# nikihowe/myriad

Hardware: AMD Instinct MI355X
Metric: converged trajopt solves/sec (batched), CARTPOLE collocation N=100 (higher is better)
Workload: dtype f64; 1 GPU; CARTPOLE HS collocation N=100, batch=4096 random x0 (weak), converged = status 0 and max|c|<=1e-8; global_batch=4096, parallelism=instances sharded over 1 GPU(s), one process per GPU

## Files before the change

myriad_amd/csrc/hs_solver_fused.h:

```cpp
#pragma once
#include <hip/hip_runtime.h>
#include "hs_solver_wave.h"

namespace myriad {

struct ParkArgs {
  int mode;
  int k1;
  const int* perm;
  const int* count;
  double* state;
  long stride;
  int fill;
  int shift;
  int* reached;
  int* cnt;
#ifdef MYR_SLOT_STAMPS
  long long* stamps;
#endif
};
constexpr int MYR_STATUS_PARKED_ = 5;
constexpr int SLOT_STAMP_WORDS = 64;

constexpr int PARK_BUCKETS = 256;
// ... 95 lines not shown
  __host__ __device__ static long off_mb(int N) { return off_hb(N) + (MLP ? (long)NodeMfma64::ntiles(npoints(N)) * NodeMfma64::HB_TILE : 0); }
  __host__ __device__ static long off_zlu(int N) { return off_mb(N) + (MLP ? (long)NodeMfma64::ntiles(npoints(N)) * NodeMfma64::MB_TILE : 0); }
  static constexpr bool FSEQ = (MYR_FWD_SEQ_NW > 0) && NW >= MYR_FWD_SEQ_NW && !MLP;
  static constexpr int FWS = NW * NW + NW;
  __host__ __device__ static long off_fw(int N) { return off_zlu(N) + (ZLU_GLOBAL ? 2L * npoints(N) * NW : 0); }
  __host__ __device__ static long scratch_doubles(int N) { return off_fw(N) + (FSEQ ? (long)N * FWS : 0); }
  static constexpr int NREC = NS + NS + NS * NS + NS * NU + NS;
  static constexpr int EXCH = NW * NW + NW * NC + NS * NC + NU * NC;
  static constexpr int NTOT = NW * NW + NW, NRED = 12;
  static constexpr int XCH = 2 * W * NREC + 2 * W * NTOT + 2 * W * 2 * NS + W * NRED + 8;
  static constexpr int NCH = W;
  static constexpr int NXB = TL ? NCH : (W > 1 ? 2 : 1);
  static constexpr int TL_TH1 = NCH * NC, TL_JN1 = (NCH - 1) * 4 * NW * NW;
  static constexpr int TL_TH = TL ? TL_TH1 + (NCH + 1) + 2 : 0, TL_JN = TL ? TL_JN1 : 0;
  __host__ __device__ static constexpr int lds_solver_doubles_z(int N, bool zlu_global) { return (zlu_global ? 2 : 4) * npoints(N) * NW + MLAM * N * NS + 6 * NW + XCH + NXB * EXCH + TL_TH + TL_JN + 8; }
  static constexpr bool ZLU_GLOBAL = (MLP && W == 2) ||
      (!MLP && (MYR_FWD_SEQ_NW > 0) && NW >= MYR_FWD_SEQ_NW && (long)lds_solver_doubles_z(100, false) * 8 > 40960L * W);
  __host__ __device__ static int lds_solver_doubles(int N) { return lds_solver_doubles_z(N, ZLU_GLOBAL); }
  __host__ __device__ static int lds_doubles(int N) { return lds_solver_doubles(N) + (MLP ? npoints(N) * NS + NodeTraits<Sys>::lds_doubles : 0); }
  __host__ __device__ static size_t lds_bytes(int N) { return (size_t)lds_doubles(N) * 8; }
  static constexpr int NSCAL = 48;
  static constexpr int PK_UNI = IpState<NS>::RECORD, PK_RES = PK_UNI + 1, PK_IT = PK_RES + 4;
  static_assert(PK_IT + 1 <= NSCAL, "record of a parked trajectory");
  __host__ __device__ static long park_doubles(int N) { return NSCAL + lds_solver_doubles(N) + (ZLU_GLOBAL ? 2L * npoints(N) * NW : 0); }

  struct Ctx {
    int N, K, n, lane, wave, tid;
    double h, h6, h8;
    double *z, *zL, *zU, *dz;
    double *hr, *st, *kg, *zr;
    double *fw;
    double *kgA, *kgB, *xA, *xB;
    double *sTh, *sJn;
    double *pt, *sF, *wl;
    double *hb, *mb;
    int nh, hidx;
    unsigned int gen;
    NodeBoard* board; int* coop_abort;
    double *pubx, *publam, *pubf;
    bool h_valid;
    const double *lb, *ub;
    bool uni;
    bool at_k1;
    SysParams<Sys> pp;
    bool term_pinned[NS];
    double *sLam, *sB, *sStash, *sTot, *sTr, *sRed, *sMisc, *sP, *sPc, *sTnu, *sKu;
#ifdef MYR_PHASE_TIMING
    long long tph[16], t0;
#endif
#ifdef MYR_TRACE
    int traj;
#endif
  };
  __device__ static inline long zi(const Ctx& c, int j, int comp) { return S::zi(c.K, j, comp); }
  __device__ static inline void use_set(Ctx& c, double* kg, double* x) {
    c.kg = kg; c.sP = x; c.sPc = x + NW * NW; c.sTnu = c.sPc + NW * NC; c.sKu = c.sTnu + NS * NC;
  }
  __device__ static inline void wsync() {
    __syncthreads();
  }
  template <int NV>
  __device__ static inline void wg_combine(Ctx& c, double* v, const int (&op)[NV]) {
    static_assert(NV <= NRED, "partial-sum slots");
    if constexpr (W > 1) {
#pragma unroll
      for (int i = 0; i < NV; ++i) c.sRed[c.wave * NRED + i] = v[i];
      __syncthreads();
#pragma unroll
      for (int i = 0; i < NV; ++i) {
        double r = c.sRed[i];
#pragma unroll
        for (int w = 1; w < W; ++w) {
          const double t = c.sRed[w * NRED + i];
          r = op[i] == 0 ? r + t : (op[i] == 1 ? (r > t ? r : t) : (r < t ? r : t));
        }
        v[i] = r;
      }
    } else { (void)c; (void)v; (void)op; }
  }

  __device__ static inline unsigned int& coop_seq(Ctx& c) { return reinterpret_cast<unsigned int*>(c.sMisc)[6]; }
  __device__ static inline unsigned int& coop_target(Ctx& c) { return reinterpret_cast<unsigned int*>(c.sMisc)[7]; }
  __device__ static inline bool coop_bounded(Ctx& c, unsigned int& spins) {
    if (++spins > MYR_COOP_SPIN_MAX || __hip_atomic_load(c.coop_abort, __ATOMIC_RELAXED, __HIP_MEMORY_SCOPE_AGENT) != 0) {
      if (spins > MYR_COOP_SPIN_MAX) __hip_atomic_store(c.coop_abort, 1, __ATOMIC_RELAXED, __HIP_MEMORY_SCOPE_AGENT);
      return true;
    }
    return false;
  }
  __device__ static inline void coop_refresh(Ctx& c) {
    if constexpr (MLP) {
      unsigned int* w = reinterpret_cast<unsigned int*>(c.sMisc) + 8;
      if (c.tid == 0) *w = __hip_atomic_load(&c.board->att, __ATOMIC_RELAXED, __HIP_MEMORY_SCOPE_AGENT) & 0xffffu;
      __syncthreads();
      const int a = __builtin_amdgcn_readfirstlane((int)*w);
      if (c.tid == 0) { COOP_TR(0, 100 + a); } if (c.tid == 64) { COOP_TR(11, 100 + a); } if (c.tid == 128) { COOP_TR(12, 100 + a); } if (c.tid == 192) { COOP_TR(13, 100 + a); }
      if (a != c.nh) { if (c.tid == 0) COOP_DBG(1, "[wg %d] owner: helpers %d -> %d\n", (int)blockIdx.x, c.nh, a); c.nh = a; c.h_valid = false; }
    } else (void)c;
  }
  template <int MODE>
  __device__ static inline void coop_post(Ctx& c, double alpha) {
    if constexpr (MLP) {
      if (MODE == 0) { for (int i = c.tid; i < c.n; i += NT) c.pubx[i] = fma(alpha, c.dz[i], c.z[i]); }
      if (MODE == 3 && !c.h_valid) { for (int i = c.tid; i < c.n; i += NT) c.pubx[i] = c.z[i]; }
      if (MODE == 4) { for (int i = c.tid; i < MLAM * c.N * NS; i += NT) c.publam[i] = c.sLam[i]; }
      if (c.tid == 0) COOP_TR(9, 1);
      coop_release();
// ... 132 lines not shown
            if (__hip_atomic_load(co.abort + 1, __ATOMIC_RELAXED, __HIP_MEMORY_SCOPE_AGENT) >= B) { quit = 1; COOP_DBG(32, "[wg %d] all finished: quit\n", (int)blockIdx.x); break; }
            __builtin_amdgcn_s_sleep(64);
            if (coop_bounded(c, spins)) { quit = 1; break; }
          }
          info[0] = found; info[1] = hid; info[2] = (int)seen; info[3] = quit | (int)(gen << 1);
          COOP_TR(5, found); COOP_TR(6, hid); COOP_TR(10, quit ? 999 : 0);
        }
        __syncthreads();
        const int found = __builtin_amdgcn_readfirstlane(info[0]), hid = __builtin_amdgcn_readfirstlane(info[1]);
        const unsigned int seen = (unsigned int)__builtin_amdgcn_readfirstlane(info[2]);
        const int quit_gen = __builtin_amdgcn_readfirstlane(info[3]);
        const int quit = quit_gen & 1;
        __syncthreads();
        if (quit) break;
        c.gen = (unsigned int)(quit_gen >> 1);
        double* so = scratch + (long)found * scratch_stride;
        c.pt = so + off_pt(c.N); c.hb = so + off_hb(c.N); c.mb = so + off_mb(c.N);
        c.board = co.boards + found; c.hidx = hid;
        c.pubx = co.pub + (long)found * co.pub_stride; c.publam = c.pubx + c.n; c.pubf = c.publam + MLAM * c.N * NS;
        coop_serve(c, seen);
      }
    } else (void)ha;
  }

  template <int MODE>
  __device__ static inline void node_pass(Ctx& c, double alpha) {
    if constexpr (MLP) {
#ifdef MYR_PHASE_TIMING
      const long long tn0_ = clock64();
#endif
      NodeMfma64::ArgsT<nd_lds> a;
      a.z = (const nd_lds*)c.z; a.dz = (const nd_lds*)c.dz; a.lam = (const nd_lds*)c.sLam; a.pt = (nd_glb*)c.pt;
      a.sF = (nd_lds*)c.sF;
      a.alpha = alpha; a.h6 = c.h6; a.h8 = c.h8; a.K = c.K; a.N = c.N;
      a.pf_f = PT_F; a.pf_a = PT_A; a.pf_b = PT_B; a.pf_d2 = PT_D2;
      a.t0 = c.wave; a.ts = W * (c.nh + 1);
      a.hb = (nd_glb*)c.hb; a.mb = (nd_glb*)c.mb; a.h_valid = c.h_valid ? 1 : 0;
      if (c.nh > 0) coop_post<MODE>(c, alpha);
      NodeMfma64::pass<MODE, nd_lds>((const nd_lds*)c.wl, a, c.lane);
      if (c.nh > 0) coop_wait<MODE>(c);
#ifdef MYR_PHASE_TIMING
      if (blockIdx.x == 0 && c.tid == 0) node_tph_[MODE] += clock64() - tn0_;
#endif
    } else { (void)c; (void)alpha; }
  }

  __device__ static inline void load_bounds(const Ctx& c, int j, double* l, double* u) {
    if (c.uni) {
      const nd_lds* b = (const nd_lds*)c.sB + ((j == 0) ? 0 : ((j == c.K - 1) ? 2 * NW : 4 * NW));
#pragma unroll
      for (int q = 0; q < NW; ++q) { l[q] = b[q]; u[q] = b[NW + q]; }
    } else {
#pragma unroll
      for (int q = 0; q < NW; ++q) { const long i = zi(c, j, q); l[q] = c.lb[i]; u[q] = c.ub[i]; }
    }
  }

  struct Step { bool on; double ap, ad, mu, ksig; };
  struct Acc { double f, cmax, cmin, sm, lg; int nm; };
  struct PRec { double x[NS], f[NS], A[NS * NS], B[NS * NU], own[NS]; };

  __device__ static inline void step_at(Ctx& c, const Step& st, int j, PRec&) {
    double bl[NW], bu[NW];
    load_bounds(c, j, bl, bu);
    const double iks = 1.0 / st.ksig;
#pragma unroll
    for (int q = 0; q < NW; ++q) {
      const long i = zi(c, j, q);
      const double l = bl[q], u = bu[q], zv = c.z[i], d = c.dz[i], zl = c.zL[i], zu = c.zU[i];
      const BoundKind k = bound_kind(l, u);
      const double zn = k.fr ? fma(st.ap, d, zv) : zv;
      const BoundMult m = bound_accept<true>(k, l, u, zv, zn, d, zl, zu, st.ad, st.mu, st.ksig, iks);
      c.z[i] = zn; c.zL[i] = m.zL; c.zU[i] = m.zU;
    }
  }

  __device__ static inline void lin_at(Ctx& c, const Step& st, int j, bool live, PRec& R, Acc& a) {
    typename S::VarBlk V;
    load_bounds(c, j, V.l, V.u);
    const double iks = 1.0 / st.ksig;
    double dv[NW];
#pragma unroll
    for (int q = 0; q < NW; ++q) {
      const long i = zi(c, j, q);
      V.z[q] = c.z[i]; V.zl[q] = c.zL[i]; V.zu[q] = c.zU[i];
      dv[q] = st.on ? c.dz[i] : 0.0;
    }
    if (st.on) {
#pragma unroll
      for (int q = 0; q < NW; ++q) {
        const long i = zi(c, j, q);
        const double l = V.l[q], u = V.u[q], zv = V.z[q], d = dv[q], zl = V.zl[q], zu = V.zu[q];
        const BoundKind k = bound_kind(l, u);
        const double zn = k.fr ? fma(st.ap, d, zv) : zv;
        const BoundMult m = bound_accept<true>(k, l, u, zv, zn, d, zl, zu, st.ad, st.mu, st.ksig, iks);
        V.z[q] = zn; V.zl[q] = m.zL; V.zu[q] = m.zU;
        if (live) { c.z[i] = V.z[q]; c.zL[i] = V.zl[q]; c.zU[i] = V.zu[q]; }
      }
    }
    double u_[NU], g, gw[NW];
#pragma unroll
    for (int q = 0; q < NS; ++q) R.x[q] = V.z[q];
#pragma unroll
    for (int q = 0; q < NU; ++q) u_[q] = V.z[NS + q];
    set_time<Sys>(c.pp.get(), tq(j, c.h));
    if constexpr (MLP) {
      const double* pt = c.pt + j;
      const int K = c.K;
#pragma unroll
      for (int q = 0; q < NS; ++q) R.f[q] = pt[(PT_F + q) * K];
#pragma unroll
      for (int q = 0; q < NS * NS; ++q) R.A[q] = pt[(PT_A + q) * K];
#pragma unroll
      for (int q = 0; q < NS * NU; ++q) R.B[q] = pt[(PT_B + q) * K];
      Sys::cost_grad(R.x, u_, c.pp.get(), &g, gw);
    } else
      Sys::lin(R.x, u_, c.pp.get(), R.f, R.A, R.B, &g, gw);
    const double wj = wq(c.K, j, c.h);
    if (TRAP && j == c.K - 1) fold_terminal<Sys>(R.x, u_, c.pp.get(), wj, g, gw);
    double cmax = a.cmax, cmin = a.cmin, sm = 0.0; int nm = 0;
    SlackLog sl;
#pragma unroll
    for (int q = 0; q < NW; ++q) {
      BoundTerms b = bound_terms(V.z[q], V.l[q], V.u[q], V.zl[q], V.zu[q], cmax, cmin);
      if (q < NS) R.own[q < NS ? q : 0] = wj * gw[q] + b.zlu;
      const BoundKind k = bound_kind(V.l[q], V.u[q]);
      mult_sum(k, V.zl[q], V.zu[q], sm, nm);
      sl.add(k, V.z[q], V.l[q], V.u[q]);
    }
    if (live) {
      a.cmax = cmax; a.cmin = cmin; a.sm += sm; a.nm += nm;
      a.lg -= sl.value();
      a.f += wj * g;
    }
  }

  struct BOut { double f, cmax, cmin, sm, lg, c1, cinf, lam_inf, sum_mult; int nm; };
  __device__ static void backward(Ctx& c, const Step& stp, const double* nuT, BOut& o) {
    using namespace detail;
    const int N = c.N, K = c.K, lane = c.lane;
    const double h6 = c.h6, h8 = c.h8;
    Acc acc{0.0, 0.0, INFINITY, 0.0, 0.0, 0};
    double c1 = 0, cinf = 0, li_ = 0, smu = 0;
    double piS[NS];
#pragma unroll
    for (int q = 0; q < NS; ++q) piS[q] = c.term_pinned[q] ? nuT[q] : 0.0;
    Step stp_ = stp;
    if constexpr (MLP) {
      if (stp.on) {
        Acc dummy{0.0, 0.0, INFINITY, 0.0, 0.0, 0};
        for (int j = c.tid; j < K; j += NT) { PRec R; step_at(c, stp, j, R); }
        (void)dummy;
        wsync();
        stp_.on = false;
      }
      node_pass<3>(c, 0.0);
      __builtin_amdgcn_fence(__ATOMIC_RELEASE, "workgroup");
      wsync();
    }
    int round = 0;
#ifdef MYR_PHASE_TIMING
    long long bw_t0_ = clock64();
#endif
    for (int r0 = N / 64; r0 >= 0; r0 -= W, ++round) {
      const int blk = r0 - c.wave;
      const int kr = blk >= 0 ? blk * 64 + 63 - lane : N + 1;
      const bool on_s = kr <= N, on = kr < N;
      const int k = on_s ? kr : N;
      PRec Rs, Rm, Re;
      lin_at(c, stp_, TRAP ? k : 2 * k, on_s, Rs, acc);
      if constexpr (!TRAP) lin_at(c, stp_, on ? 2 * k + 1 : 2 * k, on, Rm, acc);
      {
        double* rs = reinterpret_cast<double*>(&Rs); double* re = reinterpret_cast<double*>(&Re);
        double* mine = c.sStash + ((round & 1) * W + c.wave) * NREC;
        const double* theirs = c.sStash + (c.wave > 0 ? ((round & 1) * W + c.wave - 1) : (((round + 1) & 1) * W + W - 1)) * NREC;
        if (lane == 63) {
#pragma unroll
          for (int q = 0; q < NREC; ++q) mine[q] = rs[q];
        }
        wsync();
#pragma unroll
        for (int q = 0; q < NREC; ++q) {
          const double t = lane_up1(rs[q]);
          re[q] = (lane == 0) ? theirs[q] : t;
        }
      }
      MYR_BW_PH(0)
      double MA[NS * NS], Mb[NS], Ld[NS * NS], ld0[NS], Li[NS * NS], li0[NS];
      if constexpr (TRAP) {
        const double* xs = Rs.x; const double* fs = Rs.f; const double* As = Rs.A; const double* Bs = Rs.B;
        const double* xe = Re.x; const double* fe = Re.f; const double* Ae = Re.A; const double* Be = Re.B;
        const double hh = 0.5 * c.h;
        double owne[NS];
#pragma unroll
        for (int q = 0; q < NS; ++q) owne[q] = (k == N - 1 && c.term_pinned[q]) ? 0.0 : Re.own[q];
        double E[NS * NS], Ge[NS * NY1];
#pragma unroll
        for (int r = 0; r < NS; ++r) {
          const double cj = hh * (fs[r] + fe[r]) - (xe[r] - xs[r]);
          if (on) { c1 += fabs(cj); cinf = dmax(cinf, fabs(cj)); }
#pragma unroll
          for (int q = 0; q < NS; ++q) {
            E[r * NS + q] = ((r == q) ? 1.0 : 0.0) - hh * Ae[r * NS + q];
            Ge[r * NY1 + q] = ((r == q) ? 1.0 : 0.0) + hh * As[r * NS + q];
          }
#pragma unroll
          for (int a = 0; a < NU; ++a) { Ge[r * NY1 + NS + a] = hh * Bs[r * NU + a]; Ge[r * NY1 + NW + a] = hh * Be[r * NU + a]; }
          Ge[r * NY1 + NY] = cj;
        }
        lu_factor<NS>(E);
        lu_solve<NS, NY1>(E, Ge);
        if (on) {
          double* sg = c.st + (long)k * SG_N;
#pragma unroll
          for (int q = 0; q < NS * NY1; ++q) sg[SG_GE + q] = Ge[q];
        }
#pragma unroll
        for (int i = 0; i < NS; ++i) {
          double y[NS];
#pragma unroll
          for (int q = 0; q < NS; ++q) y[q] = (q == i) ? 1.0 : 0.0;
          lu_solve_t<NS>(E, y);
#pragma unroll
          for (int q = 0; q < NS; ++q) Ld[q * NS + i] = y[q];
        }
#pragma unroll
        for (int r = 0; r < NS; ++r) {
          double v = 0.0;
#pragma unroll
          for (int q = 0; q < NS; ++q) v += Ld[r * NS + q] * owne[q];
          ld0[r] = v;
          li0[r] = 0.0;
#pragma unroll
          for (int q = 0; q < NS; ++q) Li[r * NS + q] = 0.0;
        }
#pragma unroll
// ... 145 lines not shown
          for (int t = 0; t < NS; ++t) {
            const double sd = ((r == t) ? -1.0 : 0.0) - h6 * As[t * NS + r];
            const double si = ((r == t) ? -0.5 : 0.0) - h8 * As[t * NS + r];
            s += sd * (q < NS ? Ld[t * NS + q] : ld0[t]) + si * (q < NS ? Li[t * NS + q] : li0[t]);
          }
          if (q < NS) MA[r * NS + q] = on ? s : ((r == q) ? 1.0 : 0.0); else Mb[r] = on ? s : 0.0;
        }
      }
      }
      MYR_BW_PH(1)
      affine_prefix_scan_dpp<NS>(MA, Mb);
      double piN[NS];
#pragma unroll
      for (int q = 0; q < NS; ++q) piN[q] = piS[q];
      if constexpr (W > 1) {
        double* tot = c.sTot + ((round & 1) * W + c.wave) * NTOT;
        if (lane == 63) {
#pragma unroll
          for (int q = 0; q < NS * NS; ++q) tot[q] = MA[q];
#pragma unroll
          for (int q = 0; q < NS; ++q) tot[NS * NS + q] = Mb[q];
        }
        wsync();
        double pw[NS];
#pragma unroll
        for (int q = 0; q < NS; ++q) pw[q] = piS[q];
#pragma unroll
        for (int w = 0; w < W; ++w) {
          const double* tw = c.sTot + ((round & 1) * W + w) * NTOT;
          double t[NS];
#pragma unroll
          for (int r = 0; r < NS; ++r) {
            double v = tw[NS * NS + r];
#pragma unroll
            for (int q = 0; q < NS; ++q) v += tw[r * NS + q] * piN[q];
            t[r] = v;
          }
#pragma unroll
          for (int q = 0; q < NS; ++q) { piN[q] = t[q]; if (w < c.wave) pw[q] = t[q]; }
        }
#pragma unroll
        for (int q = 0; q < NS; ++q) piS[q] = pw[q];
      }
      double lo[NS], pi[NS];
#pragma unroll
      for (int r = 0; r < NS; ++r) {
        double v = Mb[r];
#pragma unroll
        for (int q = 0; q < NS; ++q) v += MA[r * NS + q] * piS[q];
        lo[r] = v;
      }
#pragma unroll
      for (int q = 0; q < NS; ++q) {
        const double t = lane_up1(lo[q]);
        pi[q] = (lane == 0) ? piS[q] : t;
      }
#pragma unroll
      for (int q = 0; q < NS; ++q) piS[q] = (W > 1) ? piN[q] : __shfl(lo[q], 63, 64);
#pragma unroll
      for (int r = 0; r < NS; ++r) {
        double d = ld0[r], i2 = li0[r];
#pragma unroll
        for (int q = 0; q < NS; ++q) { d += Ld[r * NS + q] * pi[q]; i2 += Li[r * NS + q] * pi[q]; }
        if (on) {
          c.sLam[k * NS + r] = d;
          if (!TRAP) c.sLam[N * NS + k * NS + r] = i2;
          li_ = dmax(li_, dmax(fabs(d), fabs(i2)));
          smu += fabs(d) + fabs(i2);
        }
      }
      MYR_BW_PH(2)
    }
    double v[10] = {wv_sum(acc.f), wv_max(acc.cmax), wv_min(acc.cmin), wv_sum(acc.sm), (double)wv_isum(acc.nm),
                    wv_sum(acc.lg), wv_sum(c1), wv_max(cinf), wv_max(li_), wv_sum(smu)};
    const int op[10] = {0, 1, 2, 0, 0, 0, 0, 1, 1, 0};
    wg_combine<10>(c, v, op);
    o.f = v[0]; o.cmax = v[1]; o.cmin = v[2]; o.sm = v[3]; o.nm = (int)v[4]; o.lg = v[5]; o.c1 = v[6]; o.cinf = v[7];
    o.lam_inf = v[8]; o.sum_mult = v[9];
  }

  __device__ static void hessian(Ctx& c, double& stat, double mu_fold = 0.0) {
    const int N = c.N, K = c.K;
    const double h6 = c.h6, h8 = c.h8;
    double st_ = 0;
    if constexpr (MLP) {
      node_pass<4>(c, 0.0);
      __builtin_amdgcn_fence(__ATOMIC_RELEASE, "workgroup");
      wsync();
    }
    for (int j0 = 0; j0 < K; j0 += NT) {
      const bool live = j0 + c.tid < K;
      const int j = live ? j0 + c.tid : K - 1;
      double a[NS];
      if (TRAP) {
#pragma unroll
        for (int q = 0; q < NS; ++q) {
          double s = 0.0;
          if (j >= 1) s += 0.5 * c.h * c.sLam[(j - 1) * NS + q];
          if (j < N) s += 0.5 * c.h * c.sLam[j * NS + q];
          a[q] = s;
        }
      } else if (j & 1) {
        const int k = (j - 1) >> 1;
#pragma unroll
        for (int q = 0; q < NS; ++q) a[q] = -4.0 * h6 * c.sLam[k * NS + q];
      } else {
        const int kL = (j >> 1) - 1, kR = j >> 1;
#pragma unroll
        for (int q = 0; q < NS; ++q) {
          double s = 0.0;
          if (kL >= 0) s += -h6 * c.sLam[kL * NS + q] + h8 * c.sLam[N * NS + kL * NS + q];
          if (kR < N) s += -h6 * c.sLam[kR * NS + q] - h8 * c.sLam[N * NS + kR * NS + q];
          a[q] = s;
        }
      }
      const double wj = wq(K, j, c.h);
      typename S::VarBlk V;
      load_bounds(c, j, V.l, V.u);
#pragma unroll
      for (int q = 0; q < NW; ++q) { const long i = zi(c, j, q); V.z[q] = c.z[i]; V.zl[q] = c.zL[i]; V.zu[q] = c.zU[i]; }
      HsPoint<Sys> P;
      set_time<Sys>(c.pp.get(), tq(j, c.h));
      if constexpr (MLP) {
#pragma unroll
        for (int q = 0; q < NS; ++q) P.x[q] = V.z[q];
#pragma unroll
        for (int q = 0; q < NU; ++q) P.u[q] = V.z[NS + q];
        Sys::cost_grad(P.x, P.u, c.pp.get(), &P.g, P.gw);
#pragma unroll
        for (int q = 0; q < NS * NU; ++q) P.B[q] = c.pt[(long)(PT_B + q) * K + j];
      } else
        S::lin_point(V, c.pp.get(), P);
      if (TRAP && j == K - 1) fold_terminal<Sys>(P.x, P.u, c.pp.get(), wj, P.g, P.gw);
      double sig[NW], g1v[NW], zlu[NW], cmx = 0.0, cmn = INFINITY;
#pragma unroll
      for (int q = 0; q < NW; ++q) {
        BoundTerms b = bound_terms(V.z[q], V.l[q], V.u[q], V.zl[q], V.zu[q], cmx, cmn);
        sig[q] = b.sigma; g1v[q] = b.g1; zlu[q] = b.zlu;
      }
#pragma unroll
      for (int u = 0; u < NU; ++u) {
        double r = wj * P.gw[NS + u] + zlu[NS + u];
#pragma unroll
        for (int t = 0; t < NS; ++t) r += P.B[t * NU + u] * a[t];
        st_ = live ? detail::dmax(st_, fabs(r)) : st_;
      }
      double Wh[NW * NW];
      if constexpr (MLP) {
        double Wm[NW * (NW + 1) / 2];
#pragma unroll
        for (int q = 0; q < NW * (NW + 1) / 2; ++q) Wm[q] = c.pt[(long)(PT_D2 + q) * K + j];
        Sys::hessian_packed(P.x, P.u, Wm, wj, Wh);
      } else
        Sys::hessian(P.x, P.u, c.pp.get(), P.D2, a, wj, Wh);
      double* hr = c.hr + (long)j * HR_N;
      const bool last = (j == K - 1);
      if (live) {
#pragma unroll
      for (int r = 0; r < NW; ++r) {
        const bool zr = last && r < NS && c.term_pinned[r < NS ? r : 0];
#pragma unroll
        for (int q = r; q < NW; ++q) {
          const bool zq = last && q < NS && c.term_pinned[q < NS ? q : 0];
          hr[HR_H + symidx(r, q)] = (zr || zq) ? 0.0 : (Wh[r * NW + q] + ((r == q) ? sig[r] : 0.0));
        }
        hr[HR_G0 + r] = zr ? 0.0 : (TL ? fma(mu_fold, g1v[r], wj * P.gw[r]) : wj * P.gw[r]);
        hr[HR_G1 + r] = zr ? 0.0 : g1v[r];
      }
      }
    }
    double v[1] = {wv_max(st_)};
    const int op[1] = {1};
    wg_combine<1>(c, v, op);
// ... 794 lines not shown
    }
    double* th = c.sTh + (NCH - 1) * NC;
#pragma unroll
    for (int cc = 0; cc < NC; ++cc) th[cc] = thg[cc];
  }

  __device__ static inline int knot(int k) { return TRAP ? k : 2 * k; }
  __device__ static void fwd_seq(Ctx& c, int k0, int k1) {
    constexpr int FG = 6;
    const int row = c.lane < NW ? c.lane : NW - 1;
    double x = c.dz[zi(c, knot(k0), row)];
    double ring[FG][NW + 1];
#pragma unroll
    for (int g = 0; g < FG; ++g) {
      const int k = (k0 + g < k1) ? k0 + g : k1 - 1;
      const double* f = c.fw + (long)k * FWS;
#pragma unroll
      for (int j = 0; j < NW; ++j) ring[g][j] = f[row * NW + j];
      ring[g][NW] = f[NW * NW + row];
    }
#pragma unroll 1
    for (int kb = k0; kb < k1; kb += FG) {
#pragma unroll
      for (int g = 0; g < FG; ++g) {
        const int k = kb + g;
        if (k < k1) {
          double a0 = ring[g][NW], a1 = 0.0;
#pragma unroll
          for (int j = 0; j < NW; j += 2) {
            a0 = fma(ring[g][j], rdlane(x, j), a0);
            if (j + 1 < NW) a1 = fma(ring[g][j + 1], rdlane(x, j + 1), a1);
          }
          x = a0 + a1;
          c.dz[zi(c, knot(k + 1), row)] = x;
          const int kn = (k + FG < k1) ? k + FG : k1 - 1;
          const double* f = c.fw + (long)kn * FWS;
#pragma unroll
          for (int j = 0; j < NW; ++j) ring[g][j] = f[row * NW + j];
          ring[g][NW] = f[NW * NW + row];
        }
      }
    }
  }

  __device__ static void forward(Ctx& c, const HsSolveOpts& o, double mu, const double* th, typename S::FwdOut& fo) {
    const int N = c.N, K = c.K, lane = c.lane;
    const double tau = detail::dmax(o.tau_min, 1.0 - mu);
    typename S::FwdOut l; l.alpha_p = 1.0; l.alpha_d = 1.0; l.gphi = 0.0;
    auto apply = [&](int j, const double* d, bool live) {
      typename S::VarBlk V;
      load_bounds(c, j, V.l, V.u);
      double gg, gw[NW];
#pragma unroll
      for (int q = 0; q < NW; ++q) { const long i = zi(c, j, q); V.z[q] = c.z[i]; V.zl[q] = c.zL[i]; V.zu[q] = c.zU[i]; }
      set_time<Sys>(c.pp.get(), tq(j, c.h));
      Sys::cost_grad(V.z, V.z + NS, c.pp.get(), &gg, gw);
      const double wj = wq(K, j, c.h);
      if (TRAP && j == K - 1) fold_terminal<Sys>(V.z, V.z + NS, c.pp.get(), wj, gg, gw);
      typename S::FwdOut t = l;
#pragma unroll
      for (int q = 0; q < NW; ++q) {
        if (live) c.dz[zi(c, j, q)] = d[q];
        step_limits(V.z[q], V.l[q], V.u[q], V.zl[q], V.zu[q], d[q], mu, wj * gw[q], tau, t);
      }
      if (live) l = t;
    };
    double s0[NW];
#pragma unroll
    for (int q = 0; q < NS; ++q) s0[q] = 0.0;
#pragma unroll
    for (int a = 0; a < NU; ++a) {
      double v = 0.0;
#pragma unroll
      for (int cc = 0; cc < NC; ++cc) v -= c.sKu[a * NC + cc] * th[cc];
      s0[NS + a] = v;
    }
    apply(0, s0, c.tid == 0);
    int round = 0;
    for (int base0 = 0; base0 < N; base0 += NT, ++round) {
      const int kr = base0 + c.tid;
      const bool on = kr < N;
      const int k = on ? kr : N - 1;
      const double* Kst = c.kg + (long)k * KSTR;
      const double* sg = c.st + (long)k * SG_N;
      double Kk[NQ * NW], kq[NQ], Ge[NS * NY1], Gm[TRAP ? 1 : NS * NY1];
#pragma unroll
      for (int q = 0; q < NQ * NW; ++q) Kk[q] = Kst[q];
      double thk[NC];
#pragma unroll
      for (int cc = 0; cc < NC; ++cc) thk[cc] = th[cc];
      if constexpr (TL) {
        const double* tc = c.sTh + tl_chunk(N, k) * NC;
#pragma unroll
        for (int cc = 0; cc < NC; ++cc) thk[cc] = tc[cc];
      }
#pragma unroll
      for (int t = 0; t < NQ; ++t) {
        double v = 0.0;
#pragma unroll
        for (int cc = 0; cc < NC; ++cc) v += Kst[NQ * NW + t * NC + cc] * thk[cc];
        kq[t] = v;
      }
#pragma unroll
      for (int q = 0; q < NS * NY1; ++q) { Ge[q] = sg[SG_GE + q]; if constexpr (!TRAP) Gm[q] = sg[SG_GM + q]; }
      double A[NW * NW], b[NW];
#pragma unroll
      for (int i = 0; i < NS; ++i) {
// ... 23 lines not shown
#pragma unroll
          for (int q = 0; q < NW * NW; ++q) f[q] = A[q];
#pragma unroll
          for (int q = 0; q < NW; ++q) f[NW * NW + q] = b[q];
        }
        wsync();
        if (c.wave == 0) fwd_seq(c, base0, base0 + NT < N ? base0 + NT : N);
        wsync();
#pragma unroll
        for (int q = 0; q < NW; ++q) { y[q] = c.dz[zi(c, knot(k), q)]; sn[q] = c.dz[zi(c, knot(k + 1), q)]; }
      } else {
      affine_prefix_scan_dpp<NW>(A, b);
      double sN[NW];
#pragma unroll
      for (int q = 0; q < NW; ++q) sN[q] = s0[q];
      if constexpr (W > 1) {
        double* tot = c.sTot + ((round & 1) * W + c.wave) * NTOT;
        if (lane == 63) {
#pragma unroll
          for (int q = 0; q < NW * NW; ++q) tot[q] = A[q];
#pragma unroll
          for (int q = 0; q < NW; ++q) tot[NW * NW + q] = b[q];
        }
        wsync();
        double sw[NW];
#pragma unroll
        for (int q = 0; q < NW; ++q) sw[q] = s0[q];
#pragma unroll
        for (int w = 0; w < W; ++w) {
          const double* tw = c.sTot + ((round & 1) * W + w) * NTOT;
          double t[NW];
#pragma unroll
          for (int r = 0; r < NW; ++r) {
            double v = tw[NW * NW + r];
#pragma unroll
            for (int q = 0; q < NW; ++q) v += tw[r * NW + q] * sN[q];
            t[r] = v;
          }
#pragma unroll
          for (int q = 0; q < NW; ++q) { sN[q] = t[q]; if (w < c.wave) sw[q] = t[q]; }
        }
#pragma unroll
        for (int q = 0; q < NW; ++q) s0[q] = sw[q];
      }
#pragma unroll
      for (int r = 0; r < NW; ++r) {
        double v = b[r];
#pragma unroll
        for (int q = 0; q < NW; ++q) v += A[r * NW + q] * s0[q];
        sn[r] = v;
      }
#pragma unroll
      for (int q = 0; q < NW; ++q) {
        const double t = lane_up1(sn[q]);
        y[q] = (lane == 0) ? s0[q] : t;
      }
#pragma unroll
      for (int q = 0; q < NW; ++q) s0[q] = (W > 1) ? sN[q] : __shfl(sn[q], 63, 64);
      }
#pragma unroll
      for (int t = 0; t < NQ; ++t) {
        double v = -kq[t];
#pragma unroll
        for (int q = 0; q < NW; ++q) v -= Kk[t * NW + q] * y[q];
        y[NW + t] = v;
      }
      double dm[NW], de[NW];
#pragma unroll
      for (int r = 0; r < NS; ++r) de[r] = sn[r];
#pragma unroll
      for (int a = 0; a < NU; ++a) de[NS + a] = FSEQ ? sn[NS + a] : y[NW + QE + a];
      if constexpr (TRAP) {
        (void)dm;
        apply(k + 1, de, on);
      } else {
#pragma unroll
        for (int r = 0; r < NS; ++r) {
          double vm = Gm[r * NY1 + NY];
#pragma unroll
          for (int q = 0; q < NY; ++q) vm += Gm[r * NY1 + q] * y[q];
          dm[r] = vm;
        }
#pragma unroll
        for (int a = 0; a < NU; ++a) dm[NS + a] = y[NW + a];
        apply(2 * k + 1, dm, on);
        apply(2 * k + 2, de, on);
      }
    }
    double v[3] = {wv_min(l.alpha_p), wv_min(l.alpha_d), wv_sum(l.gphi)};
    const int op[3] = {2, 2, 0};
    wg_combine<3>(c, v, op);
    fo.alpha_p = v[0]; fo.alpha_d = v[1]; fo.gphi = v[2];
  }

  struct TPt { double x[NS], f[NS]; };
  __device__ static inline void trial_point(Ctx& c, int j, double alpha, bool live, TPt& P, double& fa, double& ba, int& bad) {
    double u[NU], bl[NW], bu[NW];
    load_bounds(c, j, bl, bu);
    double slk = 1.0; int sexp = 0, bd = 0;
#pragma unroll
    for (int q = 0; q < NW; ++q) {
      const long i = zi(c, j, q);
      const double v = c.z[i] + alpha * c.dz[i];
      const double l = bl[q], ub = bu[q];
      const bool fr = l < ub;
      const bool hl = fr && (l > -INFINITY), hu = fr && (ub < INFINITY);
      const double sl = hl ? v - l : 1.0, su = hu ? ub - v : 1.0;
      bd += (sl > 0.0 ? 0 : 1) + (su > 0.0 ? 0 : 1);
      { int e_; slk *= frexp((sl > 0.0 ? sl : 1.0) * (su > 0.0 ? su : 1.0), &e_); sexp += e_; }
      if (q < NS) P.x[q < NS ? q : 0] = v; else u[q - NS] = v;
    }
    if constexpr (MLP) {
#pragma unroll
      for (int q = 0; q < NS; ++q) P.f[q] = c.sF[j * NS + q];
    } else
      Sys::f(P.x, u, c.pp.get(), P.f);
    set_time<Sys>(c.pp.get(), tq(j, c.h));
    double gj = Sys::g(P.x, u, c.pp.get());
    if (TRAP && j == c.K - 1) fold_terminal<Sys>(P.x, u, c.pp.get(), wq(c.K, j, c.h), gj, nullptr);
    if (live) {
      ba -= log(slk) + sexp * 0.6931471805599453;
      fa += wq(c.K, j, c.h) * gj;
      bad += bd;
    }
  }
  __device__ static bool trial(Ctx& c, double alpha, double mu, double& f, double& bar, double& c1) {
    const int N = c.N, lane = c.lane;
    double fa = 0, ba = 0, ca = 0; int bad = 0;
    if constexpr (MLP) {
      node_pass<0>(c, alpha);
      wsync();
    }
    TPt Pc;
    trial_point(c, 0, alpha, c.tid == 0, Pc, fa, ba, bad);
    int round = 0;
    for (int base0 = 0; base0 < N; base0 += NT, ++round) {
      const int kr = base0 + c.tid;
      const bool on = kr < N;
      const int k = on ? kr : N - 1;
      TPt Pm, Pe, Ps;
      if constexpr (!TRAP) trial_point(c, 2 * k + 1, alpha, on, Pm, fa, ba, bad);
      trial_point(c, TRAP ? k + 1 : 2 * k + 2, alpha, on, Pe, fa, ba, bad);
      if constexpr (W > 1) {
        double* mine = c.sTr + ((round & 1) * W + c.wave) * 2 * NS;
        if (lane == 63) {
#pragma unroll
          for (int q = 0; q < NS; ++q) { mine[q] = Pe.x[q]; mine[NS + q] = Pe.f[q]; }
        }
        wsync();
        if (c.wave > 0) {
          const double* theirs = c.sTr + ((round & 1) * W + c.wave - 1) * 2 * NS;
#pragma unroll
          for (int q = 0; q < NS; ++q) { Pc.x[q] = theirs[q]; Pc.f[q] = theirs[NS + q]; }
        }
      }
#pragma unroll
      for (int q = 0; q < NS; ++q) {
        const double tx = lane_up1(Pe.x[q]), tf = lane_up1(Pe.f[q]);
        Ps.x[q] = (lane == 0) ? Pc.x[q] : tx; Ps.f[q] = (lane == 0) ? Pc.f[q] : tf;
      }
      if constexpr (W > 1) {
        const double* last = c.sTr + ((round & 1) * W + W - 1) * 2 * NS;
#pragma unroll
        for (int q = 0; q < NS; ++q) { Pc.x[q] = last[q]; Pc.f[q] = last[NS + q]; }
      } else {
#pragma unroll
        for (int q = 0; q < NS; ++q) { Pc.x[q] = __shfl(Pe.x[q], 63, 64); Pc.f[q] = __shfl(Pe.f[q], 63, 64); }
      }
      if (on) {
#pragma unroll
        for (int q = 0; q < NS; ++q) {
          if constexpr (TRAP) ca += fabs(0.5 * c.h * (Ps.f[q] + Pe.f[q]) - (Pe.x[q] - Ps.x[q]));
          else {
            ca += fabs((Pe.x[q] - Ps.x[q]) - c.h6 * (Ps.f[q] + 4.0 * Pm.f[q] + Pe.f[q]));
            ca += fabs(Pm.x[q] - 0.5 * (Ps.x[q] + Pe.x[q]) - c.h8 * (Ps.f[q] - Pe.f[q]));
          }
        }
      }
    }
    double v[4] = {wv_sum(fa), wv_sum(ba), wv_sum(ca), (double)wv_isum(bad)};
    const int op[4] = {0, 0, 0, 0};
    wg_combine<4>(c, v, op);
    f = v[0]; bar = mu * v[1]; c1 = v[2];
    if (v[3] != 0.0) return false;
    if (!detail::finite_(f)) return false;
    if (!detail::finite_(c1)) return false;
    return detail::finite_(bar);
  }

  struct NuT { double v[NS]; };
  __device__ inline static BOut backward_pass(Ctx c, Step stp, NuT nu) { BOut o; backward(c, stp, nu.v, o); return o; }
  __device__ inline static double hessian_pass(Ctx c, double mu_fold) { double st; hessian(c, st, mu_fold); return st; }
  struct ThT { double v[NC]; };
  __device__ inline static typename S::FwdOut forward_pass(Ctx c, HsSolveOpts o, double mu, ThT th) { typename S::FwdOut fo; forward(c, o, mu, th.v, fo); return fo; }
  struct TrialOut { double f, bar, c1; bool ok; };
  __device__ inline static TrialOut trial_pass(Ctx c, double alpha, double mu) { TrialOut t; t.ok = trial(c, alpha, mu, t.f, t.bar, t.c1); return t; }

  __device__ static void init(Ctx& c, const double* zg) {
    const double k1 = 1e-2, k2 = 1e-2;
    const int K = c.K;
    int same = 1;
    for (int i = c.tid; i < c.n; i += NT) {
      const double l = c.lb[i], u = c.ub[i], v0 = zg[i];
      const bool fr = l < u;
      const bool hl = fr && (l > -INFINITY), hu = fr && (u < INFINITY);
      const double width = (hl && hu) ? (u - l) : INFINITY;
      const double pl = detail::dmin(k1 * detail::dmax(1.0, fabs(l)), k2 * width);
      const double pu = detail::dmin(k1 * detail::dmax(1.0, fabs(u)), k2 * width);
      double v = v0;
      v = hl ? detail::dmax(v, l + pl) : v;
      v = hu ? detail::dmin(v, u - pu) : v;
      v = fr ? v : l;
      c.z[i] = v; c.zL[i] = hl ? 1.0 : 0.0; c.zU[i] = hu ? 1.0 : 0.0;
      const int j = i < K * NS ? i / NS : (i - K * NS) / NU;
      const int q = i < K * NS ? i - j * NS : NS + (i - K * NS) - j * NU;
      if (j >= 1 && j <= K - 2) {
        const long i1 = S::zi(K, 1, q);
        const double l1 = c.lb[i1], u1 = c.ub[i1];
        same &= ((l == l1) && (u == u1)) ? 1 : 0;
      }
    }
    double sv[1] = {(double)wv_isum(same)};
    const int sop[1] = {0};
    wg_combine<1>(c, sv, sop);
    same = (sv[0] == (double)NT) ? 1 : 0;
    c.uni = __builtin_amdgcn_readfirstlane(same) != 0;
    if (c.tid < NW) {
      const int q = c.tid;
      const long i0 = S::zi(K, 0, q), iT = S::zi(K, K - 1, q), i1 = S::zi(K, 1, q);
      c.sB[q] = c.lb[i0]; c.sB[NW + q] = c.ub[i0];
      c.sB[2 * NW + q] = c.lb[iT]; c.sB[3 * NW + q] = c.ub[iT];
      c.sB[4 * NW + q] = c.lb[i1]; c.sB[5 * NW + q] = c.ub[i1];
    }
    if (c.tid < ZR) c.zr[c.tid] = 0.0;
  }

  __device__ static void solve(Ctx& c, const HsSolveOpts& o, const double* zg, HsSolveResult& res, const ParkArgs pk = ParkArgs{}, double* sv = nullptr,
                               const int* ticket = nullptr, int B = 0) {
    using namespace detail;
    const int park_mode = pk.mode, park_k1 = pk.k1;
    IpState<NS> s;
    double hist[NMMAX];
    s.start(o);
#pragma unroll
    for (int i = 0; i < NMMAX; ++i) hist[i] = 0.0;
    Step pending{false, 0.0, 0.0, 0.0, o.kappa_sigma};
    int it0 = 0;
    res.cost = 0.0; res.feas = 0.0; res.stat = 0.0; res.compl_ = 0.0;
    c.h_valid = false;
    if (park_mode == 2) {
      const int nl = lds_solver_doubles(c.N);
      for (int i = c.tid; i < nl; i += NT) c.z[i] = __builtin_nontemporal_load(&sv[NSCAL + i]);
      if constexpr (ZLU_GLOBAL) {
        for (int i = c.tid; i < 2 * c.n; i += NT) c.zL[i] = __builtin_nontemporal_load(&sv[NSCAL + nl + i]);
      }
      if (c.tid < ZR) c.zr[c.tid] = 0.0;
      s.load(sv, hist, pending);
      c.uni = sv[PK_UNI] != 0.0;
      res.cost = sv[PK_RES]; res.feas = sv[PK_RES + 1]; res.stat = sv[PK_RES + 2]; res.compl_ = sv[PK_RES + 3];
      it0 = __builtin_amdgcn_readfirstlane((int)sv[PK_IT]);
    } else
      init(c, zg);
    wsync();
#pragma unroll
    for (int q = 0; q < NS; ++q) c.term_pinned[q] = !(c.sB[2 * NW + q] < c.sB[3 * NW + q]);
    res.status = 1; res.iters = o.max_iter;
    for (int it = it0; it <= o.max_iter; ++it) {
      bool park_now = false;
// ... 279 lines not shown
    if constexpr (NWAVES > 1) {
      if (c.tid == 0) reinterpret_cast<int*>(c.sMisc)[0] = t;
      __syncthreads();
      t = reinterpret_cast<int*>(c.sMisc)[0];
    }
    long b = __builtin_amdgcn_readfirstlane(t);
    if (pk.mode == 2) {
      if (b >= pk.count[0]) break;
      b = pk.perm[b];
    } else if (b >= B) break;
    double* zg = z + b * (long)c.n;
    c.lb = lb + b * (long)c.n; c.ub = ub + b * (long)c.n;
    double* lamg = lam ? lam + b * (long)(W::MLAM * c.N * W::NS) : lam_own;
    if (poison) {
      __syncthreads();
      const unsigned int keep_seq = W::coop_seq(c), keep_target = W::coop_target(c);
      __syncthreads();
      double* l0 = reinterpret_cast<double*>(smem_fused);
      const int nl = W::lds_solver_doubles(c.N) + (W::MLP ? c.K * W::NS : 0);
      const unsigned long long salt = (unsigned long long)b * 1315423911ULL + blockIdx.x;
      for (int i = c.tid; i < nl; i += W::NT) l0[i] = poison_value(poison, (unsigned long long)i, salt);
      for (long i = c.tid; i < scratch_stride; i += W::NT) s[i] = poison_value(poison, (unsigned long long)i + (1ULL << 32), salt);
      __syncthreads();
      if (c.tid == 0) { W::coop_seq(c) = keep_seq; W::coop_target(c) = keep_target; }
      __syncthreads();
    }
#ifdef MYR_TRACE
    c.traj = (int)b;
#endif
    c.pp.load(params, b, params_stride);
    c.pp.set_scale(vs.s);
    if constexpr (W::MLP) {
      if (params_stride != 0) {
        NodeMfma64::load_weights(c.pp.get(), c.wl, c.tid, W::NT);
        __syncthreads();
      }
    }
    HsSolveResult r;
#ifdef MYR_PHASE_TIMING
    for (int i = 0; i < 16; ++i) c.tph[i] = 0;
    c.t0 = clock64();
#endif
    if constexpr (W::MLP) {
      c.nh = 0;
      c.gen = (c.gen + 1u) & MYR_COOP_GEN_MASK;
      if (coop && c.tid == 0) {
        __hip_atomic_store(&c.board->att, MYR_COOP_RUNNING | (c.gen << 16), __ATOMIC_RELAXED, __HIP_MEMORY_SCOPE_AGENT);
      }
    }
    c.at_k1 = false;
    if constexpr (NWAVES == 1 || W::MLP) W::solve(c, o, zg, r, pk, pk.state + b * pk.stride, ticket, B);
    else W::solve(c, o, zg, r);
    if (r.status != MYR_STATUS_PARKED_) {
      for (int i = c.tid; i < c.n; i += W::NT) zg[i] = c.z[i];
      for (int i = c.tid; i < W::MLAM * c.N * W::NS; i += W::NT) lamg[i] = c.sLam[i];
      if constexpr (NWAVES == 1 || W::MLP) {
        if (pk.mode == 1 && c.tid == 0) {
          pk.state[b * pk.stride + W::PK_IT] = -1.0;
          if (!c.at_k1) (void)__hip_atomic_fetch_add(pk.reached, 1, __ATOMIC_RELAXED, __HIP_MEMORY_SCOPE_AGENT);
        }
      }
    }
#ifdef MYR_SLOT_STAMPS
    if (pk.stamps && c.tid == 0) {
      long long* st_ = pk.stamps + (long)blockIdx.x * SLOT_STAMP_WORDS;
      const long long n_ = st_[2];
      if (3 + n_ < SLOT_STAMP_WORDS) st_[3 + n_] = wall_clock64();
      st_[2] = n_ + 1;
    }
#endif
#ifdef MYR_PHASE_TIMING
    if (c.lane == 0 && b < 4) {
      printf("traj %ld wave %d it %d: backward %lld hess %lld fold %lld chunk %lld wait %lld join %lld first %lld ricc %lld nu %lld forward %lld ls %lld\n",
             b, c.wave, r.iters, c.tph[0], c.tph[4], c.tph[3], c.tph[13], c.tph[5], c.tph[9], c.tph[10], c.tph[6], c.tph[7], c.tph[8], c.tph[11]);
    }
    if (!W::MLP && c.tid == 0 && blockIdx.x == 0) {
      printf("  workgroup 0, traj %ld it %d: backward pass in parts (cycles): linearisation %lld stage maps %lld scan + multipliers %lld\n", b, r.iters, bw_tph_[0], bw_tph_[1], bw_tph_[2]);
      bw_tph_[0] = bw_tph_[1] = bw_tph_[2] = 0;
    }
    if (W::MLP && c.tid == 0 && blockIdx.x == 0) {
      printf("  workgroup 0, traj %ld it %d: network passes of wavefront 0 (cycles): MODE0 %lld MODE3 %lld MODE4 %lld\n", b, r.iters, node_tph_[0], node_tph_[3], node_tph_[4]);
      node_tph_[0] = node_tph_[3] = node_tph_[4] = 0;
      for (int m = 0; m < 5; m += (m == 0 ? 3 : 1)) {
        printf("    MODE %d segments: inputs %lld | layer 1 + sigmoids %lld | layer 2 %lld | sigmoids 2 %lld | activations stored / loaded %lld | last layer %lld | tangents / contraction %lld\n", m,
               node_seg_[m][0], node_seg_[m][1], node_seg_[m][2], node_seg_[m][3], node_seg_[m][4], node_seg_[m][5], node_seg_[m][6]);
        for (int q = 0; q < 8; ++q) node_seg_[m][q] = 0;
      }
    }
#endif
    if (c.tid == 0) {
      if (cost) cost[b] = r.cost;
      if (status) status[b] = r.status;
      if (iters) iters[b] = r.iters;
      if (kkt) { kkt[3 * b] = r.feas; kkt[3 * b + 1] = r.stat; kkt[3 * b + 2] = r.compl_; }
    }
    W::wsync();
    if constexpr (W::MLP) {
      if (coop) {
        if (c.tid == 0) {
          (void)__hip_atomic_exchange(&c.board->att, 0u, __ATOMIC_RELAXED, __HIP_MEMORY_SCOPE_AGENT);
          coop_release();
          const unsigned int seq = ++W::coop_seq(c);
          __hip_atomic_store(&c.board->cmd, ((unsigned long long)seq << 32) | ((unsigned long long)c.gen << 16) | (unsigned long long)MYR_COOP_EXIT, __ATOMIC_RELAXED, __HIP_MEMORY_SCOPE_AGENT);
          coop_release();
          (void)__hip_atomic_fetch_add(co.abort + 1, 1, __ATOMIC_RELAXED, __HIP_MEMORY_SCOPE_AGENT);
        }
        c.nh = 0;
// ... 20 lines not shown
```

myriad_amd/csrc/wave_prims.h:

```cpp
#pragma once
#include <hip/hip_runtime.h>
#include "hs_solver.h"

namespace myriad {
template <bool MULTI>
__device__ inline void wave_sync() {
  if constexpr (MULTI) { __builtin_amdgcn_fence(__ATOMIC_ACQ_REL, "workgroup"); __builtin_amdgcn_wave_barrier(); }
  else __syncthreads();
}
__device__ inline double wv_sum(double v) {
#pragma unroll
  for (int o = 32; o > 0; o >>= 1) v += __shfl_xor(v, o, 64);
  return v;
}
__device__ inline double wv_max(double v) {
#pragma unroll
  for (int o = 32; o > 0; o >>= 1) { const double t = __shfl_xor(v, o, 64); v = v > t ? v : t; }
  return v;
}
__device__ inline double wv_min(double v) {
#pragma unroll
  for (int o = 32; o > 0; o >>= 1) { const double t = __shfl_xor(v, o, 64); v = v < t ? v : t; }
  return v;
}
// ... 124 lines not shown
  double A2[n * n], b2[n];
#pragma unroll
  for (int i = 0; i < n * n; ++i) A2[i] = dpp_scan_src<STEP>(A[i]);
#pragma unroll
  for (int i = 0; i < n; ++i) b2[i] = dpp_scan_src<STEP>(b[i]);
  const bool take = STEP < 4 ? (l16 >= (1 << STEP)) : (STEP == 4 ? ((lane >> 4) & 1) != 0 : lane >= 32);
  if (take) affine_after<n>(A, b, A2, b2);
}
template <int n>
__device__ inline void affine_prefix_scan_dpp(double* A, double* b) {
  affine_prefix_round<n, 0>(A, b); affine_prefix_round<n, 1>(A, b); affine_prefix_round<n, 2>(A, b);
  affine_prefix_round<n, 3>(A, b); affine_prefix_round<n, 4>(A, b); affine_prefix_round<n, 5>(A, b);
}

__device__ inline double rdlane(double v, int l) {
  int lo = __double2loint(v), hi = __double2hiint(v);
  lo = __builtin_amdgcn_readlane(lo, l);
  hi = __builtin_amdgcn_readlane(hi, l);
  return __hiloint2double(hi, lo);
}
__device__ inline double dpp_row_shr4(double v) {
  int lo = __double2loint(v), hi = __double2hiint(v), rlo, rhi;
  asm volatile("s_nop 1\n\tv_mov_b32_dpp %0, %2 row_shr:4 row_mask:0xf bank_mask:0xf bound_ctrl:1\n\t"
               "v_mov_b32_dpp %1, %3 row_shr:4 row_mask:0xf bank_mask:0xf bound_ctrl:1"
               : "=&v"(rlo), "=&v"(rhi) : "v"(lo), "v"(hi));
  return __hiloint2double(rhi, rlo);
}
__device__ inline double dpp_row_shr8(double v) {
  int lo = __double2loint(v), hi = __double2hiint(v), rlo, rhi;
  asm volatile("s_nop 1\n\tv_mov_b32_dpp %0, %2 row_shr:8 row_mask:0xf bank_mask:0xf bound_ctrl:1\n\t"
               "v_mov_b32_dpp %1, %3 row_shr:8 row_mask:0xf bank_mask:0xf bound_ctrl:1"
               : "=&v"(rlo), "=&v"(rhi) : "v"(lo), "v"(hi));
  return __hiloint2double(rhi, rlo);
}
__device__ inline void gather4(double x, double* o) {
  const auto lo = __builtin_amdgcn_permlane32_swap(__double2loint(x), __double2loint(x), false, false);
  const auto hi = __builtin_amdgcn_permlane32_swap(__double2hiint(x), __double2hiint(x), false, false);
#pragma unroll
  for (int h = 0; h < 2; ++h) {
    const auto l2 = __builtin_amdgcn_permlane16_swap(lo[h], lo[h], false, false);
    const auto h2 = __builtin_amdgcn_permlane16_swap(hi[h], hi[h], false, false);
    o[2 * h] = __hiloint2double(h2[0], l2[0]);
    o[2 * h + 1] = __hiloint2double(h2[1], l2[1]);
  }
}

template <bool ON>
__device__ inline bool uniform_if(bool c) {
  if constexpr (ON) return __builtin_amdgcn_readfirstlane((int)c) != 0;
  else return c;
}

__device__ inline double lane_up1(double v) { return __shfl_up(v, 1, 64); }

}
```

Baseline: 352,000 solves/s.

## Remap per-instance z/zL/zU into node-planar layout and use DPP lane shifts

For non-MLP systems, the per-trajectory primal and bound-multiplier arrays are re-indexed. Trapezoidal and Hermite-Simpson knots and midpoints go into separate contiguous planes, either joint or split into state and control blocks, using 32-bit indices. This aims at friendlier local memory access and cheaper address arithmetic. The final copy-out and initialisation now translate between global and local indices. Cross-lane shifts by one lane switch from __shfl_up to a wave_shr DPP move, and the lane-63 broadcast uses readlane, to avoid LDS-backed shuffle traffic. The DPP path depends on wave_shr support on the target and on correct handling of lane 0.

```diff
diff --git a/myriad_amd/csrc/hs_solver_fused.h b/myriad_amd/csrc/hs_solver_fused.h
--- a/myriad_amd/csrc/hs_solver_fused.h
+++ b/myriad_amd/csrc/hs_solver_fused.h
@@ -171,7 +171,24 @@
     int traj;
 #endif
   };
-  __device__ static inline long zi(const Ctx& c, int j, int comp) { return S::zi(c.K, j, comp); }
+  static constexpr bool LDS_PLANES = !MLP, LDS_JOINT = (NW % 2) == 1;
+  __device__ static inline int zi(const Ctx& c, int j, int comp) {
+    if constexpr (!LDS_PLANES) return (int)S::zi(c.K, j, comp);
+    else {
+      const int p = TRAP ? j : (j >> 1) + ((j & 1) ? c.N + 1 : 0);
+      if constexpr (LDS_JOINT) return p * NW + comp;
+      else return comp < NS ? p * NS + comp : c.K * NS + p * NU + (comp - NS);
+    }
+  }
+  __device__ static inline int zi_of_global(const Ctx& c, int i) {
+    if constexpr (!LDS_PLANES) return i;
+    else {
+      const int ks = c.K * NS;
+      const int j = i < ks ? i / NS : (i - ks) / NU;
+      const int q = i < ks ? i - j * NS : NS + (i - ks) - j * NU;
+      return zi(c, j, q);
+    }
+  }
   __device__ static inline void use_set(Ctx& c, double* kg, double* x) {
     c.kg = kg; c.sP = x; c.sPc = x + NW * NW; c.sTnu = c.sPc + NW * NC; c.sKu = c.sTnu + NS * NC;
   }
@@ -410,7 +427,7 @@
       for (int q = 0; q < NW; ++q) { l[q] = b[q]; u[q] = b[NW + q]; }
     } else {
 #pragma unroll
-      for (int q = 0; q < NW; ++q) { const long i = zi(c, j, q); l[q] = c.lb[i]; u[q] = c.ub[i]; }
+      for (int q = 0; q < NW; ++q) { const long i = S::zi(c.K, j, q); l[q] = c.lb[i]; u[q] = c.ub[i]; }
     }
   }
 
@@ -424,7 +441,7 @@
     const double iks = 1.0 / st.ksig;
 #pragma unroll
     for (int q = 0; q < NW; ++q) {
-      const long i = zi(c, j, q);
+      const int i = zi(c, j, q);
       const double l = bl[q], u = bu[q], zv = c.z[i], d = c.dz[i], zl = c.zL[i], zu = c.zU[i];
       const BoundKind k = bound_kind(l, u);
       const double zn = k.fr ? fma(st.ap, d, zv) : zv;
@@ -440,14 +457,14 @@
     double dv[NW];
 #pragma unroll
     for (int q = 0; q < NW; ++q) {
-      const long i = zi(c, j, q);
+      const int i = zi(c, j, q);
       V.z[q] = c.z[i]; V.zl[q] = c.zL[i]; V.zu[q] = c.zU[i];
       dv[q] = st.on ? c.dz[i] : 0.0;
     }
     if (st.on) {
 #pragma unroll
       for (int q = 0; q < NW; ++q) {
-        const long i = zi(c, j, q);
+        const int i = zi(c, j, q);
         const double l = V.l[q], u = V.u[q], zv = V.z[q], d = dv[q], zl = V.zl[q], zu = V.zu[q];
         const BoundKind k = bound_kind(l, u);
         const double zn = k.fr ? fma(st.ap, d, zv) : zv;
@@ -539,7 +556,7 @@
         wsync();
 #pragma unroll
         for (int q = 0; q < NREC; ++q) {
-          const double t = lane_up1(rs[q]);
+          const double t = lane_up1_dpp(rs[q]);
           re[q] = (lane == 0) ? theirs[q] : t;
         }
       }
@@ -791,11 +808,11 @@
       }
 #pragma unroll
       for (int q = 0; q < NS; ++q) {
-        const double t = lane_up1(lo[q]);
+        const double t = lane_up1_dpp(lo[q]);
         pi[q] = (lane == 0) ? piS[q] : t;
       }
 #pragma unroll
-      for (int q = 0; q < NS; ++q) piS[q] = (W > 1) ? piN[q] : __shfl(lo[q], 63, 64);
+      for (int q = 0; q < NS; ++q) piS[q] = (W > 1) ? piN[q] : rdlane(lo[q], 63);
 #pragma unroll
       for (int r = 0; r < NS; ++r) {
         double d = ld0[r], i2 = li0[r];
@@ -857,7 +874,7 @@
       typename S::VarBlk V;
       load_bounds(c, j, V.l, V.u);
 #pragma unroll
-      for (int q = 0; q < NW; ++q) { const long i = zi(c, j, q); V.z[q] = c.z[i]; V.zl[q] = c.zL[i]; V.zu[q] = c.zU[i]; }
+      for (int q = 0; q < NW; ++q) { const int i = zi(c, j, q); V.z[q] = c.z[i]; V.zl[q] = c.zL[i]; V.zu[q] = c.zU[i]; }
       HsPoint<Sys> P;
       set_time<Sys>(c.pp.get(), tq(j, c.h));
       if constexpr (MLP) {
@@ -1758,7 +1775,7 @@
       load_bounds(c, j, V.l, V.u);
       double gg, gw[NW];
 #pragma unroll
-      for (int q = 0; q < NW; ++q) { const long i = zi(c, j, q); V.z[q] = c.z[i]; V.zl[q] = c.zL[i]; V.zu[q] = c.zU[i]; }
+      for (int q = 0; q < NW; ++q) { const int i = zi(c, j, q); V.z[q] = c.z[i]; V.zl[q] = c.zL[i]; V.zu[q] = c.zU[i]; }
       set_time<Sys>(c.pp.get(), tq(j, c.h));
       Sys::cost_grad(V.z, V.z + NS, c.pp.get(), &gg, gw);
       const double wj = wq(K, j, c.h);
@@ -1888,7 +1905,7 @@
       }
 #pragma unroll
       for (int q = 0; q < NW; ++q) {
-        const double t = lane_up1(sn[q]);
+        const double t = lane_up1_dpp(sn[q]);
         y[q] = (lane == 0) ? s0[q] : t;
       }
 #pragma unroll
@@ -1936,7 +1953,7 @@
     double slk = 1.0; int sexp = 0, bd = 0;
 #pragma unroll
     for (int q = 0; q < NW; ++q) {
-      const long i = zi(c, j, q);
+      const int i = zi(c, j, q);
       const double v = c.z[i] + alpha * c.dz[i];
       const double l = bl[q], ub = bu[q];
       const bool fr = l < ub;
@@ -1992,7 +2009,7 @@
       }
 #pragma unroll
       for (int q = 0; q < NS; ++q) {
-        const double tx = lane_up1(Pe.x[q]), tf = lane_up1(Pe.f[q]);
+        const double tx = lane_up1_dpp(Pe.x[q]), tf = lane_up1_dpp(Pe.f[q]);
         Ps.x[q] = (lane == 0) ? Pc.x[q] : tx; Ps.f[q] = (lane == 0) ? Pc.f[q] : tf;
       }
       if constexpr (W > 1) {
@@ -2047,9 +2064,10 @@
       v = hl ? detail::dmax(v, l + pl) : v;
       v = hu ? detail::dmin(v, u - pu) : v;
       v = fr ? v : l;
-      c.z[i] = v; c.zL[i] = hl ? 1.0 : 0.0; c.zU[i] = hu ? 1.0 : 0.0;
       const int j = i < K * NS ? i / NS : (i - K * NS) / NU;
       const int q = i < K * NS ? i - j * NS : NS + (i - K * NS) - j * NU;
+      const int il = LDS_PLANES ? zi(c, j, q) : i;
+      c.z[il] = v; c.zL[il] = hl ? 1.0 : 0.0; c.zU[il] = hu ? 1.0 : 0.0;
       if (j >= 1 && j <= K - 2) {
         const long i1 = S::zi(K, 1, q);
         const double l1 = c.lb[i1], u1 = c.ub[i1];
@@ -2435,7 +2453,7 @@
     if constexpr (NWAVES == 1 || W::MLP) W::solve(c, o, zg, r, pk, pk.state + b * pk.stride, ticket, B);
     else W::solve(c, o, zg, r);
     if (r.status != MYR_STATUS_PARKED_) {
-      for (int i = c.tid; i < c.n; i += W::NT) zg[i] = c.z[i];
+      for (int i = c.tid; i < c.n; i += W::NT) zg[i] = c.z[W::zi_of_global(c, i)];
       for (int i = c.tid; i < W::MLAM * c.N * W::NS; i += W::NT) lamg[i] = c.sLam[i];
       if constexpr (NWAVES == 1 || W::MLP) {
         if (pk.mode == 1 && c.tid == 0) {
diff --git a/myriad_amd/csrc/wave_prims.h b/myriad_amd/csrc/wave_prims.h
--- a/myriad_amd/csrc/wave_prims.h
+++ b/myriad_amd/csrc/wave_prims.h
@@ -200,5 +200,12 @@
 }
 
 __device__ inline double lane_up1(double v) { return __shfl_up(v, 1, 64); }
-
-}
+__device__ inline double lane_up1_dpp(double v) {
+  int lo = __double2loint(v), hi = __double2hiint(v), rlo, rhi;
+  asm volatile("s_nop 1\n\tv_mov_b32_dpp %0, %2 wave_shr:1 row_mask:0xf bank_mask:0xf\n\t"
+               "v_mov_b32_dpp %1, %3 wave_shr:1 row_mask:0xf bank_mask:0xf"
+               : "=v"(rlo), "=v"(rhi) : "v"(lo), "v"(hi), "0"(lo), "1"(hi));
+  return __hiloint2double(rhi, rlo);
+}
+
+}
```

Result: no change. 355,000 solves/s, median of 6 (+0.9%).
